# Jamy-L/Handheld-Multi-Frame-Super-Resolution

Hardware: AMD Instinct MI355X
Metric: output Mpix/s for 12MP x 20-frame x2 SR burst; max-abs diff vs reference (higher is better)
Workload: dtype f32

## Files before the change

### handheld-multi-frame-super-resolution_amd/csrc/hhsr_pyramid.hip

```cpp
#include "hhsr_common.h"

__device__ __forceinline__ bool lp_kept(int u, int n) {
    int i = u + n / 2;
    if (i >= n) i -= n;
    return i >= n / 4 && i < n - (n + 3) / 4;
}

__global__ void __launch_bounds__(256) k_lowpass_c2c(float2* __restrict__ spec, int H, int W, int64_t sy,
                                                      int64_t sx, int xfast) {
    const int a = blockIdx.x * blockDim.x + threadIdx.x, b = blockIdx.y;
    const int x = xfast ? a : b, y = xfast ? b : a;
    if (x >= W || y >= H) return;
    if (!(lp_kept(y, H) && lp_kept(x, W))) spec[y * sy + x * sx] = make_float2(0.f, 0.f);
}

__global__ void __launch_bounds__(256) k_lowpass_r2c(float2* __restrict__ spec, int H, int W, int Wh, int64_t sy,
                                                      int64_t sx, int xfast) {
    const int a = blockIdx.x * blockDim.x + threadIdx.x, b = blockIdx.y;
    const int x = xfast ? a : b, y = xfast ? b : a;
    if (x >= Wh || y >= H) return;
    const int ny = y == 0 ? 0 : H - y, nx = x == 0 ? 0 : W - x;
    const int m = (int)(lp_kept(y, H) && lp_kept(x, W)) + (int)(lp_kept(ny, H) && lp_kept(nx, W));
    if (m == 2) return;
    float2 v = spec[y * sy + x * sx];
    const float s = 0.5f * (float)m;
    v.x *= s;
    v.y *= s;
    spec[y * sy + x * sx] = v;
}

extern "C" int hhsr_lowpass_mask_c2c(float* spec, int H, int W, int64_t stride_y, int64_t stride_x, void* stream) {
    HHSR_ARG(spec && H > 0 && W > 0 && stride_y > 0 && stride_x > 0);
    const int xfast = stride_x <= stride_y;
    const dim3 grid = xfast ? dim3(hhsr_cdiv(W, 256), H) : dim3(hhsr_cdiv(H, 256), W);
    hipLaunchKernelGGL(k_lowpass_c2c, grid, dim3(256), 0, (hipStream_t)stream, reinterpret_cast<float2*>(spec), H, W,
                       stride_y, stride_x, xfast);
    HHSR_LAUNCHED();
}

extern "C" int hhsr_lowpass_mask_r2c(float* spec, int H, int W, int64_t stride_y, int64_t stride_x, void* stream) {
    HHSR_ARG(spec && H > 0 && W > 0 && stride_y > 0 && stride_x > 0);
    const int Wh = W / 2 + 1;
    const int xfast = stride_x <= stride_y;
    const dim3 grid = xfast ? dim3(hhsr_cdiv(Wh, 256), H) : dim3(hhsr_cdiv(H, 256), Wh);
    hipLaunchKernelGGL(k_lowpass_r2c, grid, dim3(256), 0, (hipStream_t)stream, reinterpret_cast<float2*>(spec), H, W,
                       Wh, stride_y, stride_x, xfast);
    HHSR_LAUNCHED();
}

__global__ void __launch_bounds__(256) k_pad_circular(const float* __restrict__ src, int H, int W, int sp,
                                                       float* __restrict__ dst, int Hp, int Wp, int dp) {
    const int x = blockIdx.x * blockDim.x + threadIdx.x;
    const int y = blockIdx.y;
    if (x >= Wp) return;
    dst[(size_t)y * dp + x] = src[(size_t)(y % H) * sp + (x % W)];
}

extern "C" int hhsr_pad_circular(const float* src, int H, int W, int src_pitch, float* dst, int Hp, int Wp,
                                 int dst_pitch, void* stream) {
    HHSR_ARG(src && dst && H > 0 && W > 0 && Hp >= H && Wp >= W && src_pitch >= W && dst_pitch >= Wp);
    hipLaunchKernelGGL(k_pad_circular, dim3(hhsr_cdiv(Wp, 256), Hp), dim3(256), 0, (hipStream_t)stream, src, H, W,
                       src_pitch, dst, Hp, Wp, dst_pitch);
    HHSR_LAUNCHED();
}

struct Taps {
    float g[HHSR_MAX_TAPS];
};

constexpr int GD_TX = 32, GD_TY = 16;

struct GdFrames {
    const float* src[HHSR_MAX_BATCH];
    float* dst[HHSR_MAX_BATCH];
};

template <int F>
__global__ void __launch_bounds__(256) k_gauss_decimate(GdFrames fr, int H, int W, int sp,
                                                         int h2, int w2, int dp, Taps taps) {
    extern __shared__ float lds[];
    const float* __restrict__ src = fr.src[blockIdx.z];
    float* __restrict__ dst = fr.dst[blockIdx.z];
    constexpr int f = F, nt = 4 * F + 1;
    constexpr int IH = (GD_TY - 1) * f + nt, IW = (GD_TX - 1) * f + nt;
    constexpr int IWp = IW | 1;
    float* s_in = lds;
    float* s_tmp = lds + IH * IWp;
    const int bid = xcd_remap(blockIdx.y * gridDim.x + blockIdx.x, gridDim.x * gridDim.y);
    const int ox0 = (bid % gridDim.x) * GD_TX, oy0 = (bid / gridDim.x) * GD_TY;
    const int ix0 = ox0 * f, iy0 = oy0 * f;
    const int tid = threadIdx.x;
    constexpr int NL = (IH * IW + 255) / 256;
    constexpr int CH = 8;
    for (int k0 = 0; k0 < NL; k0 += CH) {
        float v[CH];
#pragma unroll
        for (int k = 0; k < CH; ++k) {
            const int p = tid + (k0 + k) * 256;
            const int r = p / IW, c = p - r * IW;
            const int y = min(iy0 + r, H - 1), x = min(ix0 + c, W - 1);
            v[k] = (k0 + k < NL && p < IH * IW) ? src[(size_t)y * sp + x] : 0.f;
        }
#pragma unroll
        for (int k = 0; k < CH; ++k) {
            const int p = tid + (k0 + k) * 256;
            if (k0 + k < NL && p < IH * IW) s_in[(p / IW) * IWp + p % IW] = v[k];
        }
    }
    __syncthreads();
    for (int p = tid; p < GD_TY * IW; p += 256) {
        const int r = p / IW, c = p - r * IW;
        float acc = 0.f;
#pragma unroll
        for (int i = 0; i < nt; ++i) acc += taps.g[i] * s_in[(r * f + i) * IWp + c];
        s_tmp[r * IWp + c] = acc;
    }
    __syncthreads();
    for (int p = tid; p < GD_TY * GD_TX; p += 256) {
        const int r = p / GD_TX, c = p - r * GD_TX;
        const int oy = oy0 + r, ox = ox0 + c;
        if (oy < h2 && ox < w2) {
            float acc = 0.f;
#pragma unroll
            for (int j = 0; j < nt; ++j) acc += taps.g[j] * s_tmp[r * IWp + c * f + j];
            dst[(size_t)oy * dp + ox] = acc;
        }
    }
}

extern "C" int hhsr_gauss_decimate_batch(const float* const* srcs, int n_frames, int H, int W, int src_pitch,
                                         float* const* dsts, int dst_pitch, int factor, const float* taps, int ntaps,
                                         void* stream) {
    HHSR_ARG(srcs && dsts && taps && n_frames >= 0 && H > 0 && W > 0 && src_pitch >= W);
    HHSR_ARG((factor == 2 || factor == 4) && ntaps == 4 * factor + 1);
    for (int n = 0; n < n_frames; ++n) HHSR_ARG(srcs[n] && dsts[n]);
    const int r = (ntaps - 1) / 2;
    const int h2 = (H - 2 * r) / factor, w2 = (W - 2 * r) / factor;
    HHSR_ARG(h2 > 0 && w2 > 0 && dst_pitch >= w2);
    Taps t;
    for (int i = 0; i < HHSR_MAX_TAPS; ++i) t.g[i] = i < ntaps ? taps[i] : 0.f;
    const int IH = (GD_TY - 1) * factor + ntaps, IWp = ((GD_TX - 1) * factor + ntaps) | 1;
    const size_t lds = (size_t)(IH + GD_TY) * IWp * sizeof(float);
    for (int n0 = 0; n0 < n_frames; n0 += HHSR_MAX_BATCH) {
        const int nb = n_frames - n0 < HHSR_MAX_BATCH ? n_frames - n0 : HHSR_MAX_BATCH;
        GdFrames fr;
        for (int k = 0; k < HHSR_MAX_BATCH; ++k) {
            fr.src[k] = srcs[n0 + (k < nb ? k : 0)];
            fr.dst[k] = dsts[n0 + (k < nb ? k : 0)];
        }
        const dim3 g(hhsr_cdiv(w2, GD_TX), hhsr_cdiv(h2, GD_TY), nb);
        if (factor == 2)
            hipLaunchKernelGGL(k_gauss_decimate<2>, g, dim3(256), lds, (hipStream_t)stream, fr, H, W, src_pitch, h2, w2,
                               dst_pitch, t);
        else
            hipLaunchKernelGGL(k_gauss_decimate<4>, g, dim3(256), lds, (hipStream_t)stream, fr, H, W, src_pitch, h2, w2,
                               dst_pitch, t);
    }
    HHSR_LAUNCHED();
}

extern "C" int hhsr_gauss_decimate(const float* src, int H, int W, int src_pitch, float* dst, int dst_pitch,
                                   int factor, const float* taps, int ntaps, void* stream) {
    HHSR_ARG(src && dst);
    return hhsr_gauss_decimate_batch(&src, 1, H, W, src_pitch, &dst, dst_pitch, factor, taps, ntaps, stream);
}
```

Measured before the change: 6313.

## Restructure Gaussian decimation to register-based vertical pass with wide tiles

Rewrites the separable Gaussian-decimate kernel so each wavefront loads input rows straight into registers (float4 loads on interior tiles) and computes the vertical filter there. Only the vertically filtered rows go to shared memory, which removes the full input tile staging and one barrier. Tiles become wider (120 or 60 outputs by 8 or 16 rows), and each lane produces several outputs from a register window. This cuts LDS traffic and index math in exchange for higher register pressure, plus a separate scalar path for edge tiles and unaligned inputs.

Result: faster. 6399 (median of 6 runs) (+1.4%).

```diff
diff --git a/handheld-multi-frame-super-resolution_amd/csrc/hhsr_pyramid.hip b/handheld-multi-frame-super-resolution_amd/csrc/hhsr_pyramid.hip
--- a/handheld-multi-frame-super-resolution_amd/csrc/hhsr_pyramid.hip
+++ b/handheld-multi-frame-super-resolution_amd/csrc/hhsr_pyramid.hip
@@ -68,64 +68,148 @@
     float g[HHSR_MAX_TAPS];
 };
 
-constexpr int GD_TX = 32, GD_TY = 16;
+template <int F>
+struct GdTile {
+    static constexpr int NT = 4 * F + 1;
+    static constexpr int TX = F == 2 ? 120 : 60;
+    static constexpr int NV = F == 2 ? 4 : 2;
+    static constexpr int TY = 4 * NV;
+    static constexpr int IW = (TX - 1) * F + NT, IH = (TY - 1) * F + NT;
+    static constexpr int NL = (IW + 3) / 4;
+    static constexpr int PW = 4 * NL;
+    static constexpr int NR = (NV - 1) * F + NT;
+    static constexpr int PO = 4 / F;
+    static constexpr int NE = (PO - 1) * F + NT;
+    static_assert(PW <= 256 && (TX * F) % 4 == 0 && TX % PO == 0 && TX / PO <= 64 && NE % 4 != 0, "tile");
+};
 
 struct GdFrames {
     const float* src[HHSR_MAX_BATCH];
     float* dst[HHSR_MAX_BATCH];
 };
 
+typedef float gd_f4 __attribute__((ext_vector_type(4)));
+
+typedef const __attribute__((address_space(1))) char* gd_gptr;
+__device__ __forceinline__ gd_gptr gd_uniform(const float* p) {
+    gd_gptr g = (gd_gptr)p;
+    asm volatile("" : "+s"(g));
+    return g;
+}
+
+typedef __attribute__((address_space(1))) char* gd_wptr;
+__device__ __forceinline__ gd_wptr gd_uniform_w(float* p) {
+    gd_wptr g = (gd_wptr)p;
+    asm volatile("" : "+s"(g));
+    return g;
+}
+
+template <int F, bool VEC>
+__device__ __forceinline__ void gd_rows(const float* __restrict__ src, int H, int W, int sp, int ix0, int ry0, bool interior,
+                                        int lane, const Taps& taps, float (*tmp)[GdTile<F>::PW]) {
+    using T = GdTile<F>;
+    float v[T::NR][4];
+    if constexpr (VEC) {
+        const unsigned lo = 16u * (unsigned)min(lane, T::NL - 1);
+#pragma unroll
+        for (int k = 0; k < T::NR; ++k) {
+            const gd_gptr rp = gd_uniform(src + (size_t)(ry0 + k) * sp + ix0);
+            const gd_f4 t = *(const __attribute__((address_space(1))) gd_f4*)(rp + lo);
+#pragma unroll
+            for (int q = 0; q < 4; ++q) v[k][q] = t[q];
+        }
+    } else {
+        unsigned lo[4];
+#pragma unroll
+        for (int q = 0; q < 4; ++q) {
+            const int c = min(lane + 64 * q, T::PW - 1);
+            lo[q] = 4u * (unsigned)(interior ? ix0 + c : min(ix0 + c, W - 1));
+        }
+#pragma unroll
+        for (int k = 0; k < T::NR; ++k) {
+            const int y = interior ? ry0 + k : min(ry0 + k, H - 1);
+            const gd_gptr rp = gd_uniform(src + (size_t)y * sp);
+#pragma unroll
+            for (int q = 0; q < 4; ++q) v[k][q] = *(const __attribute__((address_space(1))) float*)(rp + lo[q]);
+        }
+    }
+    float a[T::NV][4];
+#pragma unroll
+    for (int m = 0; m < T::NV; ++m)
+#pragma unroll
+        for (int q = 0; q < 4; ++q) {
+            float acc = 0.f;
+#pragma unroll
+            for (int i = 0; i < T::NT; ++i) acc += taps.g[i] * v[F * m + i][q];
+            a[m][q] = acc;
+        }
+    if constexpr (VEC) {
+        if (lane < T::NL)
+#pragma unroll
+            for (int m = 0; m < T::NV; ++m) {
+                gd_f4 t;
+#pragma unroll
+                for (int q = 0; q < 4; ++q) t[q] = a[m][q];
+                *reinterpret_cast<gd_f4*>(&tmp[m][4 * lane]) = t;
+            }
+    } else {
+#pragma unroll
+        for (int q = 0; q < 4; ++q)
+            if (lane + 64 * q < T::PW)
+#pragma unroll
+                for (int m = 0; m < T::NV; ++m) tmp[m][lane + 64 * q] = a[m][q];
+    }
+}
+
 template <int F>
-__global__ void __launch_bounds__(256) k_gauss_decimate(GdFrames fr, int H, int W, int sp,
-                                                         int h2, int w2, int dp, Taps taps) {
-    extern __shared__ float lds[];
+__global__ void __launch_bounds__(256) k_gauss_decimate(GdFrames fr, int H, int W, int sp, int h2, int w2, int dp,
+                                                         int vec, Taps taps) {
+    using T = GdTile<F>;
+    __shared__ __attribute__((aligned(16))) float s_tmp[T::TY][T::PW];
     const float* __restrict__ src = fr.src[blockIdx.z];
     float* __restrict__ dst = fr.dst[blockIdx.z];
-    constexpr int f = F, nt = 4 * F + 1;
-    constexpr int IH = (GD_TY - 1) * f + nt, IW = (GD_TX - 1) * f + nt;
-    constexpr int IWp = IW | 1;
-    float* s_in = lds;
-    float* s_tmp = lds + IH * IWp;
     const int bid = xcd_remap(blockIdx.y * gridDim.x + blockIdx.x, gridDim.x * gridDim.y);
-    const int ox0 = (bid % gridDim.x) * GD_TX, oy0 = (bid / gridDim.x) * GD_TY;
-    const int ix0 = ox0 * f, iy0 = oy0 * f;
-    const int tid = threadIdx.x;
-    constexpr int NL = (IH * IW + 255) / 256;
-    constexpr int CH = 8;
-    for (int k0 = 0; k0 < NL; k0 += CH) {
-        float v[CH];
-#pragma unroll
-        for (int k = 0; k < CH; ++k) {
-            const int p = tid + (k0 + k) * 256;
-            const int r = p / IW, c = p - r * IW;
-            const int y = min(iy0 + r, H - 1), x = min(ix0 + c, W - 1);
-            v[k] = (k0 + k < NL && p < IH * IW) ? src[(size_t)y * sp + x] : 0.f;
-        }
-#pragma unroll
-        for (int k = 0; k < CH; ++k) {
-            const int p = tid + (k0 + k) * 256;
-            if (k0 + k < NL && p < IH * IW) s_in[(p / IW) * IWp + p % IW] = v[k];
-        }
-    }
+    const int ox0 = (bid % gridDim.x) * T::TX, oy0 = (bid / gridDim.x) * T::TY;
+    const int ix0 = ox0 * F, iy0 = oy0 * F;
+    const int lane = threadIdx.x & 63, wv = __builtin_amdgcn_readfirstlane(threadIdx.x >> 6);
+    const bool interior = ix0 + T::PW <= W && iy0 + T::IH <= H;
+    const int ry0 = iy0 + wv * T::NV * F;
+    if (vec && interior)
+        gd_rows<F, true>(src, H, W, sp, ix0, ry0, true, lane, taps, &s_tmp[wv * T::NV]);
+    else
+        gd_rows<F, false>(src, H, W, sp, ix0, ry0, interior, lane, taps, &s_tmp[wv * T::NV]);
     __syncthreads();
-    for (int p = tid; p < GD_TY * IW; p += 256) {
-        const int r = p / IW, c = p - r * IW;
-        float acc = 0.f;
-#pragma unroll
-        for (int i = 0; i < nt; ++i) acc += taps.g[i] * s_in[(r * f + i) * IWp + c];
-        s_tmp[r * IWp + c] = acc;
-    }
-    __syncthreads();
-    for (int p = tid; p < GD_TY * GD_TX; p += 256) {
-        const int r = p / GD_TX, c = p - r * GD_TX;
-        const int oy = oy0 + r, ox = ox0 + c;
-        if (oy < h2 && ox < w2) {
+    if (lane >= T::TX / T::PO) return;
+    const int ox = ox0 + T::PO * lane;
+#pragma unroll
+    for (int p = 0; p < T::NV; ++p) {
+        const int r = wv + 4 * p, oy = oy0 + r;
+        if (oy >= h2) break;
+        float t[T::NE + 3];
+#pragma unroll
+        for (int j = 0; j < T::NE / 4; ++j) {
+            const gd_f4 u = *reinterpret_cast<const gd_f4*>(&s_tmp[r][4 * lane + 4 * j]);
+#pragma unroll
+            for (int e = 0; e < 4; ++e) t[4 * j + e] = u[e];
+        }
+#pragma unroll
+        for (int j = T::NE / 4 * 4; j < T::NE; ++j) t[j] = s_tmp[r][4 * lane + j];
+        gd_wptr rp = gd_uniform_w(dst + (size_t)oy * dp + ox0);
+#pragma unroll
+        for (int e = 0; e < T::PO; ++e) {
             float acc = 0.f;
 #pragma unroll
-            for (int j = 0; j < nt; ++j) acc += taps.g[j] * s_tmp[r * IWp + c * f + j];
-            dst[(size_t)oy * dp + ox] = acc;
-        }
-    }
+            for (int j = 0; j < T::NT; ++j) acc += taps.g[j] * t[e * F + j];
+            if (ox + e < w2) *(__attribute__((address_space(1))) float*)(rp + 4u * (unsigned)(T::PO * lane + e)) = acc;
+        }
+    }
+}
+
+template <int F>
+static void gd_launch(const GdFrames& fr, int nb, int H, int W, int sp, int h2, int w2, int dp, int vec, const Taps& t,
+                      hipStream_t stream) {
+    const dim3 g(hhsr_cdiv(w2, GdTile<F>::TX), hhsr_cdiv(h2, GdTile<F>::TY), nb);
+    hipLaunchKernelGGL(k_gauss_decimate<F>, g, dim3(256), 0, stream, fr, H, W, sp, h2, w2, dp, vec, t);
 }
 
 extern "C" int hhsr_gauss_decimate_batch(const float* const* srcs, int n_frames, int H, int W, int src_pitch,
@@ -139,22 +223,19 @@
     HHSR_ARG(h2 > 0 && w2 > 0 && dst_pitch >= w2);
     Taps t;
     for (int i = 0; i < HHSR_MAX_TAPS; ++i) t.g[i] = i < ntaps ? taps[i] : 0.f;
-    const int IH = (GD_TY - 1) * factor + ntaps, IWp = ((GD_TX - 1) * factor + ntaps) | 1;
-    const size_t lds = (size_t)(IH + GD_TY) * IWp * sizeof(float);
     for (int n0 = 0; n0 < n_frames; n0 += HHSR_MAX_BATCH) {
         const int nb = n_frames - n0 < HHSR_MAX_BATCH ? n_frames - n0 : HHSR_MAX_BATCH;
         GdFrames fr;
+        int vec = src_pitch % 4 == 0;
         for (int k = 0; k < HHSR_MAX_BATCH; ++k) {
             fr.src[k] = srcs[n0 + (k < nb ? k : 0)];
             fr.dst[k] = dsts[n0 + (k < nb ? k : 0)];
-        }
-        const dim3 g(hhsr_cdiv(w2, GD_TX), hhsr_cdiv(h2, GD_TY), nb);
+            vec = vec && ((uintptr_t)fr.src[k] & 15) == 0;
+        }
         if (factor == 2)
-            hipLaunchKernelGGL(k_gauss_decimate<2>, g, dim3(256), lds, (hipStream_t)stream, fr, H, W, src_pitch, h2, w2,
-                               dst_pitch, t);
+            gd_launch<2>(fr, nb, H, W, src_pitch, h2, w2, dst_pitch, vec, t, (hipStream_t)stream);
         else
-            hipLaunchKernelGGL(k_gauss_decimate<4>, g, dim3(256), lds, (hipStream_t)stream, fr, H, W, src_pitch, h2, w2,
-                               dst_pitch, t);
+            gd_launch<4>(fr, nb, H, W, src_pitch, h2, w2, dst_pitch, vec, t, (hipStream_t)stream);
     }
     HHSR_LAUNCHED();
 }
```
